# deepmarkpy/aware

Measured on AMD Instinct MI355X. Metric: waveform-seconds/sec through embed->attack->detect; BER vs reference, higher is better.
Workload: dtype f32 accumulation on the 16-bit MFMA pipe; conv-block GEMMs: every f32 operand scaled by a power of two and carried as TWO binary16 terms (within one f32 ulp of the operand, rms 2^-24.5), 3 partial products, the l_a*l_b term (<= 2^-22) dropped -- gemm_h2.hip: error level of an f32 dot product (agains

## Files before the change

### aware_amd/csrc/dsp_stream.hip

```cpp
#include "common.hpp"
#include "dsp_args.hpp"
#include "kernels.h"

namespace aware {

constexpr int kSW = kStreamWaves;
constexpr int kSThreads = 64 * kSW;

__device__ __forceinline__ ClipNorm clip_norm_wave(const unsigned long long* part, int nseg, int lane) {
    unsigned long long v = 0;
    for (int i = lane; i < nseg; i += 64) v = umax64(v, part[i]);
    v = wave_max64(v);
    ClipNorm c;
    const float raw = __uint_as_float((unsigned)(v >> 32));
    c.k = 0xFFFFFFFFu - (unsigned)(v & 0xFFFFFFFFu);
    c.m = raw + 1e-8f;
    c.m2 = raw / c.m + 1e-8f;
    return c;
}
__device__ __forceinline__ double dot_wave(const double* part, int nseg, int lane) {
    double s = 0.0;
    for (int i = lane; i < nseg; i += 64) s += part[i];
    return wave_sum_d(s);
}

struct LaneEnv {
    float2 lo, hi;
};
__device__ __forceinline__ LaneEnv lane_env(const PlanDev& pl, int lane) {
    LaneEnv e;
    e.lo = make_float2(fast_rcp(pl.env_tab[768 + 2 * lane]), fast_rcp(pl.env_tab[768 + 2 * lane + 1]));
    e.hi = make_float2(fast_rcp(pl.env_tab[768 + 128 + 2 * lane]), fast_rcp(pl.env_tab[768 + 128 + 2 * lane + 1]));
    return e;
}
__device__ __forceinline__ float env_at(const PlanDev& pl, int p, int T) {
    return T < 4 ? ola_envelope_loop(pl.window2, p, T) : pl.env_tab[ola_envelope_index(p, T)];
}

template <int MODE, bool L1, bool MELF = false, bool WIDE = false>
__global__ __launch_bounds__(kSThreads, MODE == AN_ADJ ? (WIDE ? 2 : 3) : 4) void analysis_stream_kernel(AnalysisArgs a, int run_frames) {
    static_assert(!(WIDE && MELF), "the wide layout takes the dense mel GEMM");
    constexpr int S = WIDE ? kFSWide : kFS;
    constexpr int NS = WIDE ? 9 : 5;
    __shared__ float magrow_s[MELF ? kSW : 1][MELF ? kFS : 1];
    __shared__ cf tw1s[512];
    __shared__ cf tw2s[64];
    __shared__ float2 wins[512];
    __shared__ cf scratch[kSW][kFftScratch];
    const int tid = threadIdx.x;
    fft_fill_tables(tid, kSThreads, a.plan.tw512, tw1s, tw2s);
    for (int i = tid; i < 512; i += kSThreads) wins[i] = make_float2(a.plan.window[2 * i], a.plan.window[2 * i + 1]);
    __syncthreads();

    int b = blockIdx.y, wgx = blockIdx.x;
    if (a.wg_tab) { const int e = a.wg_tab[blockIdx.x]; b = e >> 12; wgx = e & 4095; }
    const int f0 = a.frame_off[b];
    const int T = a.frame_off[b + 1] - f0;
    const int wave = __builtin_amdgcn_readfirstlane(tid >> 6), lane = tid & 63;
    const int t0 = (wgx * kSW + wave) * run_frames;
    if (t0 >= T) return;
    const int nfr = min(run_frames, T - t0);
    const int n = a.sig_len[b];
    const float* x = a.sig + a.sig_off[b];
    const bool al8 = (reinterpret_cast<uintptr_t>(x) & 7) == 0;

    float m = 1.f, m2 = 1.f;
    unsigned kmax = 0xFFFFFFFFu;
    if (a.pmax) {
        const ClipNorm cn = clip_norm_wave(a.pmax + (size_t)b * a.pstride, a.pcount[b], lane);
        m = cn.m;
        m2 = (MODE == AN_ADJ || a.double_norm) ? cn.m2 : 1.f;
        kmax = cn.k;
    }
    const float inv_m = 1.0f / m, inv_m2 = 1.0f / m2, inv_mm2 = 1.0f / (m * m2);
    float corr = 0.f;
    const float* gpL = nullptr;
    const float* gpR = nullptr;
    LaneEnv le;
    le.lo = le.hi = make_float2(1.f, 1.f);
    if (MODE == AN_ADJ) {
        const float adot = (float)dot_wave(a.pdot + (size_t)b * a.pstride, a.pcount[b], lane);
        const float yk = a.yraw[a.sig_off[b] + kmax];
        corr = adot * ((yk > 0.f) ? 1.f : ((yk < 0.f) ? -1.f : 0.f));
        gpL = a.gpad + (size_t)b * 1024;
        gpR = gpL + 512;
        le = lane_env(a.plan, lane);
    }

    auto load_half = [&](int P) -> float2 {
        const int s_lo = P - kHalf;
        float2 v;
        if (MODE == AN_NORM) {
            if (al8 && s_lo >= 0 && s_lo + 128 <= n) {
                v = *reinterpret_cast<const float2*>(x + s_lo + 2 * lane);
            } else {
                int s0 = s_lo + 2 * lane, s1 = s0 + 1;
                s0 = s0 < 0 ? -s0 : s0;
                s1 = s1 < 0 ? -s1 : s1;
                s0 = s0 >= n ? 2 * (n - 1) - s0 : s0;
                s1 = s1 >= n ? 2 * (n - 1) - s1 : s1;
                v.x = x[min(max(s0, 0), n - 1)];
                v.y = x[min(max(s1, 0), n - 1)];
            }
            if (a.pmax) {
                v.x = v.x * inv_m;
                v.y = v.y * inv_m;
                if (a.double_norm) { v.x = v.x * inv_m2; v.y = v.y * inv_m2; }
            }
            return v;
        }
        if (al8 && T >= 4 && s_lo >= 513 && s_lo + 127 <= n - 514 && P >= 768 && P + 127 < kHop * T) {
            float2 g = *reinterpret_cast<const float2*>(x + s_lo + 2 * lane);
            const unsigned s = (unsigned)(s_lo + 2 * lane);
            if (s == kmax) g.x -= corr;
            if (s + 1 == kmax) g.y -= corr;
            g.x = g.x * inv_mm2;
            g.y = g.y * inv_mm2;
            const float2 re = (P & 128) ? le.hi : le.lo;
            return make_float2(g.x * re.x, g.y * re.y);
        }
        float o[2];
#pragma unroll
        for (int e = 0; e < 2; ++e) {
            const int p = P + 2 * lane + e;
            const int src = p - kHalf;
            const bool valid = src >= 0 && src < n;
            float g = x[min(max(src, 0), n - 1)];
            const bool cl = src >= 1 && src <= kHalf;
            const bool cr = src >= n - kHalf - 1 && src <= n - 2;
            const float pl = gpL[min(max(kHalf - src, 0), 511)];
            const float pr = gpR[min(max(n - 2 - src, 0), 511)];
            if (cl) g += pl;
            if (cr) g += pr;
            if ((unsigned)src == kmax) g -= corr;
            g = g * inv_mm2;
            o[e] = valid ? g * fast_rcp(env_at(a.plan, p, T)) : 0.f;
        }
        return make_float2(o[0], o[1]);
    };

    cf* s = scratch[wave];
    const int band_lo = a.plan.band_lo, nband = a.plan.nband;
    cf w1024[NS];
#pragma unroll
    for (int r = 0; r < NS; ++r) w1024[r] = (r < 8) ? a.plan.tw1024[lane + 64 * r] : mk(-1.f, 0.f);
    float4 sc = make_float4(0.f, 0.f, 1.f, 0.f);
    float inv_bc2 = 1.f;
    int improved = 0;
    if (MODE == AN_ADJ && a.do_step) {
        sc = a.sched[min(max(*a.step - 1, 0), a.sched_len - 1)];
        inv_bc2 = 1.0f / sc.z;
        improved = a.improved[b];
    }

    const float l1g = (MODE == AN_ADJ && L1) ? a.l1_weight / (float)(nband * T) : 0.f;
    float wA[kMelTapsA], wB[kMelTapsB];
    int sA = 0, sB = 0;
    if (MELF) {
#pragma unroll
        for (int j = 0; j < kMelTapsA; ++j) wA[j] = a.melf_w[(size_t)lane * kMelTapsB + j];
#pragma unroll
        for (int j = 0; j < kMelTapsB; ++j) wB[j] = a.melf_w[(size_t)(lane + 64) * kMelTapsB + j];
        sA = a.melf_s[lane];
        sB = a.melf_s[lane + 64];
#pragma unroll
        for (int r = 0; r < 8; ++r) {
            const int f = lane + 64 * r - band_lo;
            if (f >= nband && f < kFS) magrow_s[MELF ? wave : 0][f] = 0.f;
        }
    }
    float2 raw[8];
#pragma unroll
    for (int r = 0; r < 8; ++r) raw[r] = load_half(kHop * t0 + 128 * r);

#pragma unroll 1
    for (int fr = 0; fr < nfr; ++fr) {
        const int t = t0 + fr;
        const size_t row = (size_t)(f0 + t);
        cf preP[NS];
        float preM[NS], preV[NS], preC[NS], pre0[NS];
        if (MODE == AN_ADJ) {
#pragma unroll
            for (int r = 0; r < NS; ++r) {
                const int f = lane + 64 * r - band_lo;
                const size_t idx = row * S + (size_t)min(max(f, 0), S - 1);
                preP[r] = a.phasor[idx];
                if (a.do_step) { preM[r] = a.mom[idx]; preV[r] = a.vel[idx]; preC[r] = a.coef[idx]; }
                else { preM[r] = preV[r] = 0.f; preC[r] = L1 ? a.coef[idx] : 0.f; }
                pre0[r] = (a.do_step || L1) ? a.c0[idx] : 0.f;
            }
        }
        cf v[8];
#pragma unroll
        for (int r = 0; r < 8; ++r) {
            const float2 w = wins[lane + 64 * r];
            v[r] = mk(raw[r].x * w.x, raw[r].y * w.y);
        }
#pragma unroll
        for (int r = 0; r < 6; ++r) raw[r] = raw[r + 2];
        raw[6] = load_half(kHop * (t + 1) + 768);
        raw[7] = load_half(kHop * (t + 1) + 896);
        fft512_wave_t<-1>(lane, v, tw1s, tw2s, s);

        const int src_lane = (64 - lane) & 63;
#pragma unroll
        for (int r = 0; r < NS; ++r) {
            cf zp = (r < 8) ? mk(__shfl(v[7 - r].x, src_lane), __shfl(v[7 - r].y, src_lane)) : v[0];
            if (lane == 0) zp = (r == 0 || r == 8) ? v[0] : v[8 - r];
            const int k = lane + 64 * r;
            const int f = k - band_lo;
            if (f < 0 || f >= nband || (r == 8 && lane != 0)) continue;
            const cf zk = v[r < 8 ? r : 0];
            const cf e = mk(0.5f * (zk.x + zp.x), 0.5f * (zk.y - zp.y));
            const cf d = mk(0.5f * (zk.x - zp.x), 0.5f * (zk.y + zp.y));
            const cf wd = cmul(w1024[r], d);
            const cf X = mk(e.x + wd.y, e.y - wd.x);
            const size_t idx = row * S + f;
            if (MODE == AN_NORM) {
                const float mg = fast_sqrt(X.x * X.x + X.y * X.y);
                const float im = fast_rcp(mg);
                if (MELF) magrow_s[wave][f] = mg;
                else if (a.mag) a.mag[idx] = mg;
                if (a.unit) a.unit[idx] = (mg > 0.f) ? mk(X.x * im, X.y * im) : mk(a.unit_default, 0.f);
            } else {
                const cf P = preP[r];
                float g = (X.x * P.x + X.y * P.y) * (1.0f / 512.0f);
                if (WIDE && (k == 0 || k == 512)) g = (X.x * P.x) * (1.0f / 1024.0f);
                if (L1) {
                    const float dc = preC[r] - pre0[r];
                    g += l1g * ((dc > 0.f) ? 1.f : ((dc < 0.f) ? -1.f : 0.f));
                }
                if (a.grad_out) a.grad_out[idx] = g;
                if (a.do_step) {
                    float mo = preM[r], ve = preV[r], p = preC[r];
                    float blo, bhi;
                    box_bounds(pre0[r], a.box_ratio, blo, bhi);
                    nadam_clamp_update(p, mo, ve, g, blo, bhi, sc.x, sc.y, inv_bc2, a.hyp);
                    a.mom[idx] = mo; a.vel[idx] = ve; a.coef[idx] = p;
                    if (improved) a.best[idx] = p;
                }
            }
        }
        if (MODE == AN_NORM && MELF) {
            float* mr = magrow_s[MELF ? wave : 0];
            float m0 = 0.f, m1 = 0.f;
#pragma unroll
            for (int j = 0; j < kMelTapsA; ++j) m0 += wA[j] * mr[sA + j];
#pragma unroll
            for (int j = 0; j < kMelTapsB; ++j) m1 += wB[j] * mr[sB + j];
            float* mo = a.mel_out + row * 128;
            mo[lane] = m0;
            mo[lane + 64] = m1;
        }
        if (MODE == AN_NORM && a.write_pad) {
            if (WIDE) {
                for (int f = nband + lane; f < S; f += 64) {
                    const size_t idx = row * S + f;
                    if (a.mag) a.mag[idx] = 0.f;
                    if (a.unit) a.unit[idx] = mk(0.f, 0.f);
                }
            } else {
#pragma unroll
                for (int r = 0; r < 8; ++r) {
                    const int f = lane + 64 * r - band_lo;
                    if (f >= nband && f < kFS) {
                        const size_t idx = row * kFS + f;
                        if (a.mag) a.mag[idx] = 0.f;
                        if (a.unit) a.unit[idx] = mk(0.f, 0.f);
                    }
                }
            }
        }
    }
}

template <int MODE, bool L1, bool MELG = false, bool WIDE = false>
__global__ __launch_bounds__(kSThreads, WIDE ? 3 : 4) void synth_stream_kernel(SynthArgs a) {
    static_assert(!(WIDE && MELG), "the wide layout takes the dense mel GEMM");
    constexpr int S = WIDE ? kFSWide : kFS;
    constexpr int NS = WIDE ? 9 : 8;
    __shared__ float2 melw_s[MELG ? kFS : 1];
    __shared__ float melrow_s[MELG ? kSW : 1][MELG ? 128 : 1];
    __shared__ cf tw1s[512];
    __shared__ cf tw2s[64];
    __shared__ float2 wins[512];
    __shared__ cf mcs[512];
    __shared__ cf scratch[kSW][kFftScratch];
    const int tid = threadIdx.x;
    const float scale = (MODE == SY_FWD) ? (1.0f / 512.0f) : 1.0f;
    fft_fill_tables(tid, kSThreads, a.plan.tw512, tw1s, tw2s);
    for (int i = tid; i < 512; i += kSThreads) {
        wins[i] = make_float2(a.plan.window[2 * i] * scale, a.plan.window[2 * i + 1] * scale);
        const cf w = a.plan.tw1024[i];
        mcs[i] = (WIDE || i < 256) ? mk(0.5f * (1.f + w.y), 0.5f * w.x) : mk(0.5f * (1.f - w.y), -0.5f * w.x);
    }
    if (MELG)
        for (int i = tid; i < kFS; i += kSThreads) melw_s[i] = a.melw[i];
    __syncthreads();

    int b = blockIdx.y, wgx = blockIdx.x;
    if (a.wg_tab) { const int e = a.wg_tab[blockIdx.x]; b = e >> 12; wgx = e & 4095; }
    const int f0 = a.frame_off[b];
    const int T = a.frame_off[b + 1] - f0;
    const int nblk = T - 1;
    const int wave = __builtin_amdgcn_readfirstlane(tid >> 6), lane = tid & 63;
    const int run = wgx * kSW + wave;
    int nseg, jb0, jb1;
    synth_segment(nblk, run, a.run_blocks, nseg, jb0, jb1);
    if (run >= nseg || T < 1) return;
    const bool first = jb0 == 0, last = jb1 == nblk;
    const int t_lo = max(jb0 - 1, 0);
    const int t_hi = (MODE == SY_ADJ && last) ? T + 2 : jb1 + 1;
    const int Ny = kHop * nblk;
    const int so = sig_offset(a.frame_off, b);
    float* out = a.out + so;
    const float* add = (MODE == SY_FWD && a.add) ? a.add + so : nullptr;
    const float* y = (MODE == SY_ADJ) ? a.yraw + so : nullptr;
    float inv_m = 1.f, inv_m2 = 1.f;
    if (MODE == SY_ADJ) {
        const ClipNorm cn = clip_norm_wave(a.pmax_in + (size_t)b * a.pstride, a.pcount[b], lane);
        inv_m = 1.0f / cn.m;
        inv_m2 = 1.0f / cn.m2;
    }
    const LaneEnv le = lane_env(a.plan, lane);
    const int band_lo = a.plan.band_lo, nband = a.plan.nband;
    cf* s = scratch[wave];

    float inA[NS];
    cf inP[NS];
    unsigned fo[NS];
    unsigned inband = 0;
#pragma unroll
    for (int r = 0; r < NS; ++r) {
        const int k = lane + 64 * r;
        const int f = (WIDE ? k : ((k <= 256) ? k : 512 - k)) - band_lo;
        fo[r] = (unsigned)min(max(f, 0), S - 1);
        if (f >= 0 && f < nband && !(r == 8 && lane != 0)) inband |= 1u << r;
    }
    unsigned mtap[2] = {0u, 0u};
    float drow[2] = {0.f, 0.f};
    if (MELG) {
#pragma unroll
        for (int r = 0; r < 8; ++r) mtap[r >> 2] |= (unsigned)a.melm[fo[r]] << (8 * (r & 3));
    }
    auto load_band = [&](int t) {
        const size_t row = (size_t)(f0 + t);
        const float* A = MELG ? nullptr : a.amp + row * S;
        const cf* P = a.ph + row * S;
        if (MELG) {
            const float* D = a.dmel + row * 128;
            drow[0] = D[lane];
            drow[1] = D[lane + 64];
        }
#pragma unroll
        for (int r = 0; r < NS; ++r) {
            inP[r] = P[fo[r]];
            if (!MELG) {
                const float am = A[fo[r]];
                inA[r] = ((inband >> r) & 1u) ? am : 0.f;
            }
        }
    };
    auto expand_mel = [&]() {
        float* mr = melrow_s[MELG ? wave : 0];
        mr[lane] = drow[0];
        mr[lane + 64] = drow[1];
#pragma unroll
        for (int r = 0; r < 8; ++r) {
            const unsigned m = (mtap[r >> 2] >> (8 * (r & 3))) & 0xFFu;
            const float2 w = melw_s[MELG ? fo[r] : 0];
            const float v = w.x * mr[m] + w.y * mr[m + 1];
            inA[r] = ((inband >> r) & 1u) ? v : 0.f;
            if (r == 3) __builtin_amdgcn_sched_barrier(0);
        }
    };

    float2 acc[6];
#pragma unroll
    for (int q = 0; q < 6; ++q) acc[q] = make_float2(0.f, 0.f);
    unsigned long long best = 0;
    double dot = 0.0;
    float l1 = 0.f;
    if (t_lo <= T - 1) load_band(t_lo);

    auto epi_operands = [&](int i, bool emit, float2& e0, float2& e1) {
        e0 = make_float2(0.f, 0.f);
        e1 = e0;
        if (emit) {
            const float* src = (MODE == SY_FWD) ? add : y;
            if (src) {
                e0 = *reinterpret_cast<const float2*>(src + kHop * i + 2 * lane);
                e1 = *reinterpret_cast<const float2*>(src + kHop * i + 128 + 2 * lane);
            }
        }
    };
    auto ola_emit = [&](int i, bool emit, const float2 (&c)[8], const float2 e0, const float2 e1) {
        const float2 o0 = make_float2(acc[0].x + c[0].x, acc[0].y + c[0].y);
        const float2 o1 = make_float2(acc[1].x + c[1].x, acc[1].y + c[1].y);
#pragma unroll
        for (int q = 0; q < 4; ++q) acc[q] = make_float2(acc[q + 2].x + c[q + 2].x, acc[q + 2].y + c[q + 2].y);
        acc[4] = c[6];
        acc[5] = c[7];

        const int j0 = kHop * i + 2 * lane, j1 = j0 + 128;
        if (MODE == SY_FWD) {
            if (emit) {
                float2 r0, r1;
                if (T >= 4 && i >= 1 && i <= T - 3) { r0 = le.lo; r1 = le.hi; }
                else {
                    r0 = make_float2(fast_rcp(env_at(a.plan, kHalf + j0, T)), fast_rcp(env_at(a.plan, kHalf + j0 + 1, T)));
                    r1 = make_float2(fast_rcp(env_at(a.plan, kHalf + j1, T)), fast_rcp(env_at(a.plan, kHalf + j1 + 1, T)));
                }
                float2 v0 = make_float2(o0.x * r0.x, o0.y * r0.y), v1 = make_float2(o1.x * r1.x, o1.y * r1.y);
                if (add) { v0.x += e0.x; v0.y += e0.y; v1.x += e1.x; v1.y += e1.y; }
                *reinterpret_cast<float2*>(out + j0) = v0;
                *reinterpret_cast<float2*>(out + j1) = v1;
                best = umax64(best, pack_max(fabsf(v0.x), (unsigned)j0));
                best = umax64(best, pack_max(fabsf(v0.y), (unsigned)j0 + 1));
                best = umax64(best, pack_max(fabsf(v1.x), (unsigned)j1));
                best = umax64(best, pack_max(fabsf(v1.y), (unsigned)j1 + 1));
            }
        } else {
            if (emit) {
                *reinterpret_cast<float2*>(out + j0) = o0;
                *reinterpret_cast<float2*>(out + j1) = o1;
                dot += (double)o0.x * (double)((e0.x * inv_m) * inv_m2) + (double)o0.y * (double)((e0.y * inv_m) * inv_m2);
                dot += (double)o1.x * (double)((e1.x * inv_m) * inv_m2) + (double)o1.y * (double)((e1.y * inv_m) * inv_m2);
            } else if (first && i < 0 && i >= -2) {
                float* gp = a.gpad + (size_t)b * 1024;
                const int p0 = kHop * (i + 2) + 2 * lane, p1 = p0 + 128;
                *reinterpret_cast<float2*>(gp + p0) = o0;
                *reinterpret_cast<float2*>(gp + p1) = o1;
                const float ov[4] = {o0.x, o0.y, o1.x, o1.y};
                const int pp[4] = {p0, p0 + 1, p1, p1 + 1};
#pragma unroll
                for (int e = 0; e < 4; ++e) {
                    const int j = kHalf - pp[e];
                    const float yv = y[min(max(j, 0), max(Ny - 1, 0))];
                    if (j >= 1 && j < Ny) dot += (double)ov[e] * (double)((yv * inv_m) * inv_m2);
                }
            } else if (last && i >= nblk && i <= nblk + 1) {
                float* gp = a.gpad + (size_t)b * 1024 + 512;
                const int u0 = kHop * (i - nblk) + 2 * lane, u1 = u0 + 128;
                *reinterpret_cast<float2*>(gp + u0) = o0;
                *reinterpret_cast<float2*>(gp + u1) = o1;
                const float ov[4] = {o0.x, o0.y, o1.x, o1.y};
                const int uu[4] = {u0, u0 + 1, u1, u1 + 1};
#pragma unroll
                for (int e = 0; e < 4; ++e) {
                    const int j = Ny - 2 - uu[e];
                    const float yv = y[min(max(j, 0), max(Ny - 1, 0))];
                    if (j >= 0) dot += (double)ov[e] * (double)((yv * inv_m) * inv_m2);
                }
            }
        }
    };

    const int t_fft = min(t_hi, T - 1);
#pragma unroll 1
    for (int t = t_lo; t <= t_fft; ++t) {
        const int i = t - 2;
        const bool emit = i >= jb0 && i < jb1;
        float2 e0, e1;
        epi_operands(i, emit, e0, e1);
        float2 c[8];
        {
            if (MELG) expand_mel();
            if (MODE == SY_FWD && L1 && ((t >= jb0 && t < jb1) || (last && t == T - 1))) {
                const float* C0 = a.c0 + (size_t)(f0 + t) * S;
#pragma unroll
                for (int r = 0; r < (WIDE ? NS : 5); ++r) {
                    const int f = lane + 64 * r - band_lo;
                    const float cv = C0[min(max(f, 0), S - 1)];
                    if (f >= 0 && f < nband && (WIDE ? (r < 8 || lane == 0) : (r < 4 || lane == 0))) l1 += fabsf(inA[r] - cv);
                }
            }
            cf v[8];
            if (WIDE) {
                cf xo[NS];
#pragma unroll
                for (int r = 0; r < NS; ++r) {
                    const bool edge = (r == 0 || r == 8) && lane == 0;
                    xo[r] = mk(inA[r] * inP[r].x, edge ? 0.f : inA[r] * inP[r].y);
                    if (MODE == SY_ADJ && edge) xo[r].x *= 2.f;
                }
                const int src_lane = (64 - lane) & 63;
#pragma unroll
                for (int r = 0; r < 8; ++r) {
                    cf xp = mk(__shfl(xo[7 - r].x, src_lane), __shfl(xo[7 - r].y, src_lane));
                    if (lane == 0) xp = xo[8 - r];
                    const cf A = mcs[lane + 64 * r];
                    const cf Bm = mk(1.f - A.x, -A.y);
                    const cf xk = xo[r];
                    v[r] = mk(xk.x * A.x - xk.y * A.y + xp.x * Bm.x + xp.y * Bm.y,
                              xk.x * A.y + xk.y * A.x + xp.x * Bm.y - xp.y * Bm.x);
                }
            } else {
#pragma unroll
            for (int r = 0; r < 8; ++r) {
                const cf mc = mcs[lane + 64 * r];
                const float xr = inA[r] * inP[r].x, xi = (r < 4) ? inA[r] * inP[r].y : -(inA[r] * inP[r].y);
                v[r] = mk(xr * mc.x - xi * mc.y, xr * mc.y + xi * mc.x);
            }
            }
            load_band(min(t + 1, T - 1));
            fft512_wave_t<1>(lane, v, tw1s, tw2s, s);
#pragma unroll
            for (int r = 0; r < 8; ++r) {
                const float2 w = wins[lane + 64 * r];
                c[r] = make_float2(v[r].x * w.x, v[r].y * w.y);
            }
        }
        ola_emit(i, emit, c, e0, e1);
    }
#pragma unroll 1
    for (int t = t_fft + 1; t <= t_hi; ++t) {
        const int i = t - 2;
        const bool emit = i >= jb0 && i < jb1;
        float2 e0, e1;
        epi_operands(i, emit, e0, e1);
        float2 c[8];
#pragma unroll
        for (int r = 0; r < 8; ++r) c[r] = make_float2(0.f, 0.f);
        ola_emit(i, emit, c, e0, e1);
    }
    if (MODE == SY_FWD) {
        if (a.pmax) {
            best = wave_max64(best);
            if (lane == 0) a.pmax[(size_t)b * a.pstride + run] = best;
        }
        if (L1) {
            const double tot = wave_sum_d((double)l1);
            if (lane == 0) a.pl1[(size_t)b * a.pstride + run] = tot;
        }
    } else {
        dot = wave_sum_d(dot);
        if (lane == 0) a.pdot[(size_t)b * a.pstride + run] = dot;
    }
}

__global__ __launch_bounds__(64) void l1_reduce_kernel(const double* __restrict__ pl1, const int* __restrict__ pcount, int pstride,
                                                        const int* __restrict__ frame_off, int nband, float weight,
                                                        float* __restrict__ l1term) {
    const int b = blockIdx.x, lane = threadIdx.x;
    const double s = dot_wave(pl1 + (size_t)b * pstride, pcount[b], lane);
    const int T = frame_off[b + 1] - frame_off[b];
    if (lane == 0) l1term[b] = weight * (float)(s / (double)(nband * T));
}
void launch_l1_reduce(const double* pl1, const int* pcount, int pstride, const int* frame_off, int nband, float weight,
                      float* l1term, int B, hipStream_t st) {
    hipLaunchKernelGGL(l1_reduce_kernel, dim3(B), dim3(64), 0, st, pl1, pcount, pstride, frame_off, nband, weight, l1term);
}

bool stream_supported(const PlanDev& plan) {
    return plan.stride == kFSWide || (plan.band_lo >= 1 && plan.band_lo + plan.nband <= 257);
}

void launch_analysis_stream(const AnalysisLaunch& L, hipStream_t st) {
    AnalysisArgs a{};
    a.plan = L.plan;
    a.frame_off = L.frame_off;
    a.sig = L.sig; a.sig_off = L.sig_off; a.sig_len = L.sig_len;
    a.pmax = L.pmax; a.pcount = L.pcount; a.pstride = L.pstride;
    a.double_norm = L.double_norm; a.unit_default = L.unit_default;
    a.mag = L.mag; a.unit = (cf*)L.unit; a.full = nullptr;
    a.yraw = L.yraw; a.pdot = L.pdot; a.phasor = (const cf*)L.phasor;
    a.coef = L.coef; a.mom = L.mom; a.vel = L.vel; a.lo = L.lo; a.hi = L.hi; a.best = L.best;
    a.improved = L.improved; a.sched = (const float4*)L.sched; a.sched_len = L.sched_len > 0 ? L.sched_len : 1; a.step = L.step;
    a.grad_out = L.grad_out; a.do_step = L.do_step;
    a.hyp = make_float4(L.hyp[0], L.hyp[1], L.hyp[2], L.hyp[3]);
    a.gpad = L.gpad; a.write_pad = L.write_pad;
    a.c0 = L.c0; a.box_ratio = L.box_ratio; a.l1_weight = L.l1_weight;
    int R = 4;
    dim3 grid;
    if (L.run_frames >= 4 && L.run_frames <= 16 && L.wg_tab && L.n_wg > 0) {
        R = L.run_frames;
        a.wg_tab = L.wg_tab;
        grid = dim3((unsigned)L.n_wg, 1, 1);
    } else {
        for (int cand = 16; cand >= 4; --cand)
            if ((long)L.B * ((L.max_frames + cand - 1) / cand) >= 4096) { R = cand; break; }
        for (int cand = R; cand >= 4 && cand >= R - 3; --cand)
            if (((L.max_frames + cand - 1) / cand) % kSW == 0) { R = cand; break; }
        const int runs = (L.max_frames + R - 1) / R;
        grid = dim3((unsigned)((runs + kSW - 1) / kSW), (unsigned)L.B, 1);
    }
    if (L.plan.stride == kFSWide) {
        if (L.adjoint && a.l1_weight != 0.f) hipLaunchKernelGGL((analysis_stream_kernel<AN_ADJ, true, false, true>), grid, dim3(kSThreads), 0, st, a, R);
        else if (L.adjoint) hipLaunchKernelGGL((analysis_stream_kernel<AN_ADJ, false, false, true>), grid, dim3(kSThreads), 0, st, a, R);
        else hipLaunchKernelGGL((analysis_stream_kernel<AN_NORM, false, false, true>), grid, dim3(kSThreads), 0, st, a, R);
    } else if (L.adjoint && a.l1_weight != 0.f) hipLaunchKernelGGL((analysis_stream_kernel<AN_ADJ, true>), grid, dim3(kSThreads), 0, st, a, R);
    else if (L.adjoint) hipLaunchKernelGGL((analysis_stream_kernel<AN_ADJ, false>), grid, dim3(kSThreads), 0, st, a, R);
    else if (L.mel_out && L.melf_w && L.melf_s) {
        a.mel_out = L.mel_out; a.melf_w = L.melf_w; a.melf_s = L.melf_s; a.mag = nullptr;
        hipLaunchKernelGGL((analysis_stream_kernel<AN_NORM, false, true>), grid, dim3(kSThreads), 0, st, a, R);
    } else hipLaunchKernelGGL((analysis_stream_kernel<AN_NORM, false>), grid, dim3(kSThreads), 0, st, a, R);
}

void launch_synth_stream(const SynthLaunch& L, hipStream_t st) {
    SynthArgs a{};
    a.plan = L.plan;
    a.frame_off = L.frame_off;
    a.amp = L.amp; a.ph = (const cf*)L.ph; a.full = nullptr;
    a.out = L.out; a.add = L.add; a.pmax = L.pmax; a.pstride = L.pstride;
    a.yraw = L.yraw; a.pmax_in = L.pmax_in; a.pcount = L.pcount; a.pdot = L.pdot; a.gpad = L.gpad;
    a.c0 = L.c0; a.pl1 = (L.c0 && L.pl1) ? L.pl1 : nullptr;
    const int nblk = L.max_frames - 1;
    a.run_blocks = (L.run_blocks >= 1 && L.run_blocks <= kSynthBlocks) ? L.run_blocks : kSynthBlocks;
    int runs = (nblk + a.run_blocks - 1) / a.run_blocks;
    if (runs < 1) runs = 1;
    dim3 grid((unsigned)((runs + kSW - 1) / kSW), (unsigned)L.B, 1);
    if (L.wg_tab && L.n_wg > 0 && a.run_blocks == L.run_blocks) {
        a.wg_tab = L.wg_tab;
        grid = dim3((unsigned)L.n_wg, 1, 1);
    }
    a.dmel = L.dmel; a.melw = (const float2*)L.melw; a.melm = L.melm;
    if (L.plan.stride == kFSWide) {
        if (L.adjoint) hipLaunchKernelGGL((synth_stream_kernel<SY_ADJ, false, false, true>), grid, dim3(kSThreads), 0, st, a);
        else if (a.pl1) hipLaunchKernelGGL((synth_stream_kernel<SY_FWD, true, false, true>), grid, dim3(kSThreads), 0, st, a);
        else hipLaunchKernelGGL((synth_stream_kernel<SY_FWD, false, false, true>), grid, dim3(kSThreads), 0, st, a);
    } else if (L.adjoint && L.dmel && L.melw && L.melm) hipLaunchKernelGGL((synth_stream_kernel<SY_ADJ, false, true>), grid, dim3(kSThreads), 0, st, a);
    else if (L.adjoint) hipLaunchKernelGGL((synth_stream_kernel<SY_ADJ, false>), grid, dim3(kSThreads), 0, st, a);
    else if (a.pl1) hipLaunchKernelGGL((synth_stream_kernel<SY_FWD, true>), grid, dim3(kSThreads), 0, st, a);
    else hipLaunchKernelGGL((synth_stream_kernel<SY_FWD, false>), grid, dim3(kSThreads), 0, st, a);
}

}
```

Before: 1939.

## Vectorize optimizer state updates through LDS gradient row; pack mel taps

In the adjoint analysis kernel, per-bin gradients are staged in the wave's FFT scratch as a row. The NAdam moment, velocity, coef and c0 arrays are then loaded and stored as float4 in contiguous lane order instead of strided scalar accesses. In the synth kernel, mel tap index and weights are packed into one 16-byte shared struct, and the per-lane column offsets are recomputed on the fly instead of held in registers. This is meant to improve global coalescing and cut register pressure, at the cost of an extra LDS round trip, a wave sync, and the assumption that rows are 16-byte aligned.

```diff
diff --git a/aware_amd/csrc/dsp_stream.hip b/aware_amd/csrc/dsp_stream.hip
--- a/aware_amd/csrc/dsp_stream.hip
+++ b/aware_amd/csrc/dsp_stream.hip
@@ -42,11 +42,13 @@
     static_assert(!(WIDE && MELF), "the wide layout takes the dense mel GEMM");
     constexpr int S = WIDE ? kFSWide : kFS;
     constexpr int NS = WIDE ? 9 : 5;
+    constexpr int NQ = (S / 4 + 63) / 64;
+    static_assert(S % 4 == 0 && S <= 2 * kFftScratch, "gradient row in the FFT scratch");
     __shared__ float magrow_s[MELF ? kSW : 1][MELF ? kFS : 1];
     __shared__ cf tw1s[512];
     __shared__ cf tw2s[64];
     __shared__ float2 wins[512];
-    __shared__ cf scratch[kSW][kFftScratch];
+    __shared__ __align__(16) cf scratch[kSW][kFftScratch];
     const int tid = threadIdx.x;
     fft_fill_tables(tid, kSThreads, a.plan.tw512, tw1s, tw2s);
     for (int i = tid; i < 512; i += kSThreads) wins[i] = make_float2(a.plan.window[2 * i], a.plan.window[2 * i + 1]);
@@ -140,6 +142,7 @@
     };
 
     cf* s = scratch[wave];
+    float* grow = reinterpret_cast<float*>(s);
     const int band_lo = a.plan.band_lo, nband = a.plan.nband;
     cf w1024[NS];
 #pragma unroll
@@ -178,16 +181,26 @@
         const int t = t0 + fr;
         const size_t row = (size_t)(f0 + t);
         cf preP[NS];
-        float preM[NS], preV[NS], preC[NS], pre0[NS];
+        float4 qM[NQ], qV[NQ], qC[NQ], q0[NQ];
         if (MODE == AN_ADJ) {
 #pragma unroll
             for (int r = 0; r < NS; ++r) {
                 const int f = lane + 64 * r - band_lo;
-                const size_t idx = row * S + (size_t)min(max(f, 0), S - 1);
-                preP[r] = a.phasor[idx];
-                if (a.do_step) { preM[r] = a.mom[idx]; preV[r] = a.vel[idx]; preC[r] = a.coef[idx]; }
-                else { preM[r] = preV[r] = 0.f; preC[r] = L1 ? a.coef[idx] : 0.f; }
-                pre0[r] = (a.do_step || L1) ? a.c0[idx] : 0.f;
+                preP[r] = a.phasor[row * S + (size_t)min(max(f, 0), S - 1)];
+            }
+            const float4 z4 = make_float4(0.f, 0.f, 0.f, 0.f);
+#pragma unroll
+            for (int q = 0; q < NQ; ++q) {
+                const size_t i4 = row * (S / 4) + (size_t)min(lane + 64 * q, S / 4 - 1);
+                if (a.do_step) {
+                    qM[q] = reinterpret_cast<const float4*>(a.mom)[i4];
+                    qV[q] = reinterpret_cast<const float4*>(a.vel)[i4];
+                    qC[q] = reinterpret_cast<const float4*>(a.coef)[i4];
+                } else {
+                    qM[q] = qV[q] = z4;
+                    qC[q] = L1 ? reinterpret_cast<const float4*>(a.coef)[i4] : z4;
+                }
+                q0[q] = (a.do_step || L1) ? reinterpret_cast<const float4*>(a.c0)[i4] : z4;
             }
         }
         cf v[8];
@@ -226,18 +239,58 @@
                 const cf P = preP[r];
                 float g = (X.x * P.x + X.y * P.y) * (1.0f / 512.0f);
                 if (WIDE && (k == 0 || k == 512)) g = (X.x * P.x) * (1.0f / 1024.0f);
-                if (L1) {
-                    const float dc = preC[r] - pre0[r];
-                    g += l1g * ((dc > 0.f) ? 1.f : ((dc < 0.f) ? -1.f : 0.f));
-                }
-                if (a.grad_out) a.grad_out[idx] = g;
-                if (a.do_step) {
-                    float mo = preM[r], ve = preV[r], p = preC[r];
-                    float blo, bhi;
-                    box_bounds(pre0[r], a.box_ratio, blo, bhi);
-                    nadam_clamp_update(p, mo, ve, g, blo, bhi, sc.x, sc.y, inv_bc2, a.hyp);
-                    a.mom[idx] = mo; a.vel[idx] = ve; a.coef[idx] = p;
-                    if (improved) a.best[idx] = p;
+                grow[f] = g;
+            }
+        }
+        if (MODE == AN_ADJ) {
+            wave_sync();
+#pragma unroll
+            for (int q = 0; q < NQ; ++q) {
+                const int c4 = min(lane + 64 * q, S / 4 - 1);
+                const float4 g4 = reinterpret_cast<const float4*>(grow)[c4];
+                const float gq[4] = {g4.x, g4.y, g4.z, g4.w};
+                float mq[4] = {qM[q].x, qM[q].y, qM[q].z, qM[q].w};
+                float vq[4] = {qV[q].x, qV[q].y, qV[q].z, qV[q].w};
+                float cq[4] = {qC[q].x, qC[q].y, qC[q].z, qC[q].w};
+                const float zq[4] = {q0[q].x, q0[q].y, q0[q].z, q0[q].w};
+                const int f4 = 4 * (lane + 64 * q);
+                const size_t i4 = row * (S / 4) + c4;
+                float gv[4];
+#pragma unroll
+                for (int e = 0; e < 4; ++e) {
+                    float g = gq[e];
+                    if (L1) {
+                        const float dc = cq[e] - zq[e];
+                        g += l1g * ((dc > 0.f) ? 1.f : ((dc < 0.f) ? -1.f : 0.f));
+                    }
+                    gv[e] = g;
+                    if (a.do_step) {
+                        float blo, bhi;
+                        box_bounds(zq[e], a.box_ratio, blo, bhi);
+                        nadam_clamp_update(cq[e], mq[e], vq[e], g, blo, bhi, sc.x, sc.y, inv_bc2, a.hyp);
+                    }
+                }
+                if (f4 + 3 < nband) {
+                    if (a.grad_out)
+#pragma unroll
+                        for (int e = 0; e < 4; ++e) a.grad_out[row * S + f4 + e] = gv[e];
+                    if (a.do_step) {
+                        reinterpret_cast<float4*>(a.mom)[i4] = make_float4(mq[0], mq[1], mq[2], mq[3]);
+                        reinterpret_cast<float4*>(a.vel)[i4] = make_float4(vq[0], vq[1], vq[2], vq[3]);
+                        reinterpret_cast<float4*>(a.coef)[i4] = make_float4(cq[0], cq[1], cq[2], cq[3]);
+                        if (improved) reinterpret_cast<float4*>(a.best)[i4] = make_float4(cq[0], cq[1], cq[2], cq[3]);
+                    }
+                } else if (f4 < nband) {
+#pragma unroll
+                    for (int e = 0; e < 4; ++e) {
+                        if (f4 + e >= nband) continue;
+                        const size_t idx = row * S + f4 + e;
+                        if (a.grad_out) a.grad_out[idx] = gv[e];
+                        if (a.do_step) {
+                            a.mom[idx] = mq[e]; a.vel[idx] = vq[e]; a.coef[idx] = cq[e];
+                            if (improved) a.best[idx] = cq[e];
+                        }
+                    }
                 }
             }
         }
@@ -274,12 +327,17 @@
     }
 }
 
+struct __align__(16) MelTap {
+    float x, y;
+    unsigned m, pad;
+};
+
 template <int MODE, bool L1, bool MELG = false, bool WIDE = false>
 __global__ __launch_bounds__(kSThreads, WIDE ? 3 : 4) void synth_stream_kernel(SynthArgs a) {
     static_assert(!(WIDE && MELG), "the wide layout takes the dense mel GEMM");
     constexpr int S = WIDE ? kFSWide : kFS;
     constexpr int NS = WIDE ? 9 : 8;
-    __shared__ float2 melw_s[MELG ? kFS : 1];
+    __shared__ MelTap melw_s[MELG ? kFS : 1];
     __shared__ float melrow_s[MELG ? kSW : 1][MELG ? 128 : 1];
     __shared__ cf tw1s[512];
     __shared__ cf tw2s[64];
@@ -295,7 +353,7 @@
         mcs[i] = (WIDE || i < 256) ? mk(0.5f * (1.f + w.y), 0.5f * w.x) : mk(0.5f * (1.f - w.y), -0.5f * w.x);
     }
     if (MELG)
-        for (int i = tid; i < kFS; i += kSThreads) melw_s[i] = a.melw[i];
+        for (int i = tid; i < kFS; i += kSThreads) melw_s[i] = MelTap{a.melw[i].x, a.melw[i].y, a.melm[i], 0u};
     __syncthreads();
 
     int b = blockIdx.y, wgx = blockIdx.x;
@@ -328,21 +386,16 @@
 
     float inA[NS];
     cf inP[NS];
-    unsigned fo[NS];
+    const int cb_lo = lane - band_lo, cb_hi = 512 - lane - band_lo;
+    auto col = [&](int r) -> int { return min(max((WIDE || r < 4) ? cb_lo + 64 * r : cb_hi - 64 * r, 0), S - 1); };
     unsigned inband = 0;
 #pragma unroll
     for (int r = 0; r < NS; ++r) {
         const int k = lane + 64 * r;
         const int f = (WIDE ? k : ((k <= 256) ? k : 512 - k)) - band_lo;
-        fo[r] = (unsigned)min(max(f, 0), S - 1);
         if (f >= 0 && f < nband && !(r == 8 && lane != 0)) inband |= 1u << r;
     }
-    unsigned mtap[2] = {0u, 0u};
     float drow[2] = {0.f, 0.f};
-    if (MELG) {
-#pragma unroll
-        for (int r = 0; r < 8; ++r) mtap[r >> 2] |= (unsigned)a.melm[fo[r]] << (8 * (r & 3));
-    }
     auto load_band = [&](int t) {
         const size_t row = (size_t)(f0 + t);
         const float* A = MELG ? nullptr : a.amp + row * S;
@@ -354,9 +407,10 @@
         }
 #pragma unroll
         for (int r = 0; r < NS; ++r) {
-            inP[r] = P[fo[r]];
+            const int fo = col(r);
+            inP[r] = P[fo];
             if (!MELG) {
-                const float am = A[fo[r]];
+                const float am = A[fo];
                 inA[r] = ((inband >> r) & 1u) ? am : 0.f;
             }
         }
@@ -367,8 +421,8 @@
         mr[lane + 64] = drow[1];
 #pragma unroll
         for (int r = 0; r < 8; ++r) {
-            const unsigned m = (mtap[r >> 2] >> (8 * (r & 3))) & 0xFFu;
-            const float2 w = melw_s[MELG ? fo[r] : 0];
+            const MelTap w = melw_s[MELG ? col(r) : 0];
+            const unsigned m = w.m;
             const float v = w.x * mr[m] + w.y * mr[m + 1];
             inA[r] = ((inband >> r) & 1u) ? v : 0.f;
             if (r == 3) __builtin_amdgcn_sched_barrier(0);
```

After: 1964, median of 6. 1.01x the previous value.
